# translearn/PaintRL

Measured on NVIDIA B200. Metric: batched env steps/sec, higher is better.
Workload: dtype f64

## Files before the change

### paintrl_b200/csrc/paintrl_capi.cu

```cuda
#include <algorithm>
#include <cmath>
#include <cstdio>
#include <cstring>
#include <numeric>
#include <string>
#include <vector>

#include "../../include/paintrl.h"
#include "paintrl_kernels.cuh"
#include "paintrl_raster.cuh"
#include "paintrl_param.cuh"
#include "paintrl_policy.cuh"
#include "paintrl_learn.cuh"

using namespace paintrl;

static const int kFusedBelowEnvs = 16384;

namespace {

thread_local std::string g_error;

int fail(int code, const std::string &msg) {
    g_error = msg;
// ... 47 lines not shown
        if (e == cudaSuccess) ptrs.push_back(*out);
        return e;
    }
    size_t static_bytes() const {
        size_t n = 0;
        for (const Slab &s : slabs) n += s.used;
        return n;
    }
};

}

struct PaintrlEngine {
    int device = 0;
    int num_envs = 0;
    int color = 0;
    DevPack pk{};
    DevConfig cfg{};
    DeviceArena arena;
    EnvState *states = nullptr;
    MoveOut *moves = nullptr;
    EnvStat *env_stats = nullptr;
    unsigned *bits = nullptr;
    int16_t *thick = nullptr;
    unsigned *grid_cnt = nullptr;
    unsigned long long *stats = nullptr;
    ShotPoses *shots = nullptr;
    unsigned *last_mask = nullptr;
    bool paint_normal = false;
    unsigned *ready = nullptr;
    int carveout_percent = -1;
    bool carveout_set = false;
    bool carveout_set_subset = false;
    void *stage_actions = nullptr;
    unsigned char *stage_out = nullptr;
    void *slot_actions[2] = {nullptr, nullptr};
    unsigned char *slot_out[2] = {nullptr, nullptr};
    cudaStream_t copy_in = nullptr, copy_out = nullptr;
    cudaEvent_t ev_in[2] = {nullptr, nullptr}, ev_step[2] = {nullptr, nullptr}, ev_done[2] = {nullptr, nullptr};
    bool slot_pending[2] = {false, false};
    unsigned long long launches = 0;
    double move_cell_planes_mean = 0.0, move_cell_verts_mean = 0.0;
    int move_lanes = 32;
    int move_warps = 4, paint_warps = 1;
    int move_minb = 4;
    void *cold_args = nullptr;
    int fused = -1;
    bool move_fast = true;
    bool force_unstaged = false;
};

namespace {

bool host_ray(const PaintrlPartPack *pack, const double *frm, const double *d, double *t_hit, int *arg_in = nullptr,
              int *arg_out = nullptr) {
    double t_in = -INFINITY, t_out = INFINITY;
    int ai = -1, ao = -1;
    bool outside = false;
    for (int i = 0; i < pack->n_planes; ++i) {
        const double *n = pack->plane_n + 3 * i;
        double den = n[0] * d[0] + n[1] * d[1] + n[2] * d[2];
        double num = pack->plane_off[i] - (n[0] * frm[0] + n[1] * frm[1] + n[2] * frm[2]);
        if (den == 0.0) {
            if (num < 0.0) { outside = true; if (ai < 0) ai = i; }
            continue;
        }
// ... 629 lines not shown
    }
    return PAINTRL_OK;
}

template <bool SUBSET>
int launch_step(PaintrlHandle h, const EnvSel &sel, const StepIO &io, void *stream) {
    const int n = sel.n;
    const void *actions_dev = io.actions;
    bool &carveout_done = SUBSET ? h->carveout_set_subset : h->carveout_set;
    CUDA_TRY(cudaSetDevice(h->device));
    if (h->paint_normal) {
        cudaStream_t ns = as_stream(stream);
        const int threads = 128;
        move_kernel<32, 4, false, SUBSET><<<(n * 32 + threads - 1) / threads, threads, 0, ns>>>(h->pk, h->cfg, env_arrays(h), h->num_envs, actions_dev, sel);
        int rc = launch_check(h, "move_kernel");
        if (rc != PAINTRL_OK) return rc;
        if (h->color == 0) paint_normal_kernel<0, SUBSET><<<n, 32, 0, ns>>>(h->pk, h->cfg, env_arrays(h), h->num_envs, io, (const ColdArgs *)h->cold_args, sel);
        else paint_normal_kernel<1, SUBSET><<<n, 32, 0, ns>>>(h->pk, h->cfg, env_arrays(h), h->num_envs, io, (const ColdArgs *)h->cold_args, sel);
        cudaError_t nerr = cudaGetLastError();
        if (nerr != cudaSuccess) {
            cudaMemsetAsync(h->ready, 0, sizeof(unsigned) * (size_t)h->num_envs, ns);
            return fail(PAINTRL_E_CUDA, std::string("paint_normal_kernel: ") + cudaGetErrorString(nerr));
        }
        h->launches++;
        return PAINTRL_OK;
    }
    const bool use_fused = h->fused >= 0 ? h->fused == 1 : n < kFusedBelowEnvs;
    if (use_fused) {
        const bool staged_f = h->pk.n_words_pad <= kStageWords && !h->force_unstaged;
        const bool ax12f = h->pk.axis0 == 1 && h->pk.axis1 == 2, disc = h->cfg.action_mode == 0;
        const EnvArrays fea = env_arrays(h);
        const ColdArgs *cold = (const ColdArgs *)h->cold_args;
        cudaStream_t fs = as_stream(stream);
#define PAINTRL_FUSED_K(C, ST, AX, DI) step_fused_kernel<C, ST, AX, DI, SUBSET><<<(n + PAINTRL_FUSED_WPB - 1) / PAINTRL_FUSED_WPB, 32 * PAINTRL_FUSED_WPB, 0, fs>>>(h->pk, h->cfg, fea, h->num_envs, io, cold, sel)
#define PAINTRL_FUSED_AD(C, ST)                                                        \
    do {                                                                               \
        if (ax12f && disc) PAINTRL_FUSED_K(C, ST, true, true);                         \
        else if (ax12f) PAINTRL_FUSED_K(C, ST, true, false);                           \
        else if (disc) PAINTRL_FUSED_K(C, ST, false, true);                            \
        else PAINTRL_FUSED_K(C, ST, false, false);                                     \
    } while (0)
        if (h->color == 0) { if (staged_f) PAINTRL_FUSED_AD(0, true); else PAINTRL_FUSED_AD(0, false); }
        else { if (staged_f) PAINTRL_FUSED_AD(1, true); else PAINTRL_FUSED_AD(1, false); }
#undef PAINTRL_FUSED_AD
#undef PAINTRL_FUSED_K
        return launch_check(h, "step_fused_kernel");
    }
    {
        const int threads = h->move_warps * 32;
        cudaStream_t ms = as_stream(stream);
        const int L = h->move_lanes;
        const int mblocks = (int)(((long long)n * L + threads - 1) / threads);
        const bool ax12m = h->pk.axis0 == 1 && h->pk.axis1 == 2;
#define PAINTRL_MOVE(G, MINB)                                                                                              \
    do {                                                                                                                   \
        if (!carveout_done && h->carveout_percent >= 0) {                                                                \
            cudaFuncSetAttribute(move_kernel<G, MINB, true, SUBSET>, cudaFuncAttributePreferredSharedMemoryCarveout, h->carveout_percent);  \
            cudaFuncSetAttribute(move_kernel<G, MINB, false, SUBSET>, cudaFuncAttributePreferredSharedMemoryCarveout, h->carveout_percent); \
        }                                                                                                                  \
        if (ax12m) move_kernel<G, MINB, true, SUBSET><<<mblocks, threads, 0, ms>>>(h->pk, h->cfg, env_arrays(h), h->num_envs, actions_dev, sel);  \
        else move_kernel<G, MINB, false, SUBSET><<<mblocks, threads, 0, ms>>>(h->pk, h->cfg, env_arrays(h), h->num_envs, actions_dev, sel);       \
    } while (0)
#define PAINTRL_MOVE_FAST(G)                                                                                               \
    do {                                                                                                                   \
        if (ax12m && discrete) move_fast_kernel<G, true, true, SUBSET><<<mblocks, threads, 0, ms>>>(h->pk, h->cfg, env_arrays(h), h->num_envs, actions_dev, sel);   \
        else if (ax12m) move_fast_kernel<G, true, false, SUBSET><<<mblocks, threads, 0, ms>>>(h->pk, h->cfg, env_arrays(h), h->num_envs, actions_dev, sel);         \
        else if (discrete) move_fast_kernel<G, false, true, SUBSET><<<mblocks, threads, 0, ms>>>(h->pk, h->cfg, env_arrays(h), h->num_envs, actions_dev, sel);      \
        else move_fast_kernel<G, false, false, SUBSET><<<mblocks, threads, 0, ms>>>(h->pk, h->cfg, env_arrays(h), h->num_envs, actions_dev, sel);                   \
    } while (0)
        const bool discrete = h->cfg.action_mode == 0;
        if (h->move_fast) {
            if (L == 8) PAINTRL_MOVE_FAST(8); else if (L == 16) PAINTRL_MOVE_FAST(16); else PAINTRL_MOVE_FAST(32);
        } else if (h->move_minb == 7) {
            if (L == 8) PAINTRL_MOVE(8, 7); else if (L == 16) PAINTRL_MOVE(16, 7); else PAINTRL_MOVE(32, 7);
        } else {
            if (L == 8) PAINTRL_MOVE(8, 4); else if (L == 16) PAINTRL_MOVE(16, 4); else PAINTRL_MOVE(32, 4);
        }
#undef PAINTRL_MOVE_FAST
// ... 944 lines not shown
```

### paintrl_b200/csrc/paintrl_kernels.cuh

```cuda
#pragma once
#include "paintrl_device.cuh"

namespace paintrl {

struct StepIO {
    const void *actions;
    double *obs, *reward, *penalty, *actual;
    uint8_t *done;
    int32_t *new_texels;
    double *next_obs;
    const int32_t *reset_start_idx;
};

struct EnvSel {
    const int32_t *ids;
    int lo, n;
};

template <bool SUBSET>
__device__ __forceinline__ bool step_env(const EnvSel &sel, int k, int num_envs, int &env) {
    if (!SUBSET) { env = k; return k < num_envs; }
    if (k >= sel.n) return false;
    env = sel.ids ? __ldg(&sel.ids[k]) : sel.lo + k;
    return (unsigned)env < (unsigned)num_envs;
// ... 382 lines not shown
#pragma unroll
        for (int s = 0; s <= NS; ++s) in |= (ball_exact(ws, x, y, z, s) ? 1u : 0u) << s;
    } else {
#pragma unroll
        for (int s = 0; s <= NS; ++s) in |= (e[s] <= 0.f ? 1u : 0u) << s;
    }
    if (!has_last) in &= (1u << NS) - 1u;
    return in;
}

template <typename WS>
__device__ __forceinline__ void ball_flags_at(const DevPack &pk, const ShotsF &c, const WS &ws, int j, float tx, float ty, float tz,
                                              bool has_last, bool &any_shot, bool &possible) {
    float e[NS + 1];
    bool in[NS + 1];
    if (ball_pretest_at(c, tx, ty, tz, e)) {
        const double x = __ldg(&pk.tx[j]), y = __ldg(&pk.ty[j]), z = __ldg(&pk.tz[j]);
#pragma unroll
        for (int s = 0; s <= NS; ++s) in[s] = ball_exact(ws, x, y, z, s);
    } else {
#pragma unroll
        for (int s = 0; s <= NS; ++s) in[s] = e[s] <= 0.f;
    }
    bool prev = has_last && in[NS];
    any_shot = false;
    possible = false;
#pragma unroll
    for (int s = 0; s < NS; ++s) {
        any_shot = any_shot || in[s];
        possible = possible || (in[s] && !prev);
        prev = in[s];
    }
}
template <typename WS>
__device__ __forceinline__ void ball_flags(const DevPack &pk, const ShotsF &c, const WS &ws, int j, bool has_last, bool &any_shot,
                                           bool &possible) {
    ball_flags_at(pk, c, ws, j, __ldg(&pk.fx[j]), __ldg(&pk.fy[j]), __ldg(&pk.fz[j]), has_last, any_shot, possible);
}

template <bool STAGED, int COLOR, typename WS>
__device__ __forceinline__ int stamp_ranges(const DevPack &pk, float lo0, float hi0, float lo1, float hi1, int lane, WS &ws) {
    const float rr = (float)kPaintRadius + 4e-5f;
    int base = 0;
    for (int r0 = 0; r0 < pk.n_rows; r0 += 32) {
        const int r = r0 + lane;
        int wa = 0, wn = 0;
        if (r < pk.n_rows) {
            const float ylo = fmaf((float)r, pk.rel_row_h, pk.rel_row_o1) - 2e-5f, yhi = ylo + pk.rel_row_h + 4e-5f;
            const float dy = fmaxf(0.f, fmaxf(ylo - hi1, lo1 - yhi));
            if (dy <= rr) {
                const float hw = sqrtf(rr * rr - dy * dy) + 4e-5f;
                const float fa = floorf((lo0 - hw - pk.rel_cx_o0) * pk.rel_cx_inv) - 1.f;
                const float fb = floorf((hi0 + hw - pk.rel_cx_o0) * pk.rel_cx_inv) + 1.f;
                if (fb >= 0.f && fa < (float)pk.ncx) {
                    const int ca = (int)fmaxf(fa, 0.f), cb = (int)fminf(fb, (float)(pk.ncx - 1));
                    const int *cs = pk.cell_start + (size_t)r * (pk.ncx + 1);
                    const int i0 = __ldg(cs + ca), i1 = __ldg(cs + cb + 1);
                    if (i1 > i0) {
                        wa = __ldg(&pk.row_word0[r]) + (i0 >> 5);
                        wn = ((i1 - 1) >> 5) - (i0 >> 5) + 1;
                    }
                }
            }
            ws.rowWa[r] = wa;
            ws.rowWn[r] = wn;
        }
        if (STAGED) {
            int incl = wn;
#pragma unroll
            for (int o = 1; o < 32; o <<= 1) {
                const int u = __shfl_up_sync(kFull, incl, o);
                if (lane >= o) incl += u;
            }
            const int at = base + incl - wn;
            for (int t = 0; t < wn; ++t) ws.cand[at + t] = (uint16_t)(wa + t);
            base += __shfl_sync(kFull, incl, 31);
        }
    }
    __syncwarp();
    return base;
}

template <bool STAGED, typename WS, typename BodyFn>
__device__ __forceinline__ void for_each_stamp_word(const DevPack &pk, int lane, const WS &ws, int n_cand, BodyFn body) {
    if constexpr (STAGED) {
        for (int k = 0; k < n_cand; ++k) body((int)ws.cand[k]);
    } else {
        for (int r0 = 0; r0 < pk.n_rows; r0 += 32) {
            const int r = r0 + lane;
            const int wa = r < pk.n_rows ? ws.rowWa[r] : 0, wn = r < pk.n_rows ? ws.rowWn[r] : 0;
            unsigned m = __ballot_sync(kFull, wn > 0);
            while (m) {
                const int src = __ffs(m) - 1;
                m &= m - 1;
                const int a = __shfl_sync(kFull, wa, src), n = __shfl_sync(kFull, wn, src);
                for (int w = a; w < a + n; ++w) body(w);
            }
        }
    }
}

template <int COLOR, bool STAGED, typename WS, typename BITS>
__device__ __forceinline__ void stamp(const DevPack &pk, const Ax &ax, const BITS &bits, int16_t *thick, unsigned *grid_cnt, bool has_last,
                                      int lane, WS &ws, int &n_new_out, int &n_possible_out, bool &dirty_out PAINTRL_PROF_PARAM) {
    ShotsF c;
#pragma unroll
    for (int s = 0; s <= NS; ++s) {
        c.x[s] = (float)(cen(ws, s, 0) - pk.org0);
        c.y[s] = (float)(cen(ws, s, 1) - pk.org1);
        c.z[s] = (float)(cen(ws, s, 2) - pk.org2);
    }
    float lo0 = INFINITY, hi0 = -INFINITY, lo1 = INFINITY, hi1 = -INFINITY;
#pragma unroll
    for (int s = 0; s < NS; ++s) {
        const float c0 = ax.a0 == 0 ? c.x[s] : (ax.a0 == 1 ? c.y[s] : c.z[s]);
        const float c1 = ax.a1 == 0 ? c.x[s] : (ax.a1 == 1 ? c.y[s] : c.z[s]);
        lo0 = fminf(lo0, c0); hi0 = fmaxf(hi0, c0);
        lo1 = fminf(lo1, c1); hi1 = fmaxf(hi1, c1);
    }
    PAINTRL_PROF(17, lane == 0);
    const int n_cand = stamp_ranges<STAGED, COLOR>(pk, lo0, hi0, lo1, hi1, lane, ws);
    PAINTRL_PROF(18, lane == 0);

    double rmax[NS];
    if (COLOR == 1) {
#pragma unroll
        for (int s = 0; s < NS; ++s) rmax[s] = -1.0;
        for_each_stamp_word<STAGED>(pk, lane, ws, n_cand, [&](int w) {
            const int j = w * 32 + lane;
            const unsigned in = ball_mask(pk, c, ws, j, false);
            if (in) {
                const double x = __ldg(&pk.tx[j]), y = __ldg(&pk.ty[j]), z = __ldg(&pk.tz[j]);
#pragma unroll
                for (int s = 0; s < NS; ++s) {
                    if (in & (1u << s)) {
                        const double dx = x - cen(ws, s, 0), dy = y - cen(ws, s, 1), dz = z - cen(ws, s, 2);
                        rmax[s] = fmax(rmax[s], dx * dx + dy * dy + dz * dz);
                    }
                }
            }
        });
#pragma unroll
        for (int s = 0; s < NS; ++s) rmax[s] = sqrt(warp_max(rmax[s]));
        if (lane < NS) {
// ... 19 lines not shown
                m &= m - 1;
                const int a = __shfl_sync(kFull, wa, src), n = __shfl_sync(kFull, wn, src);
                for (int w0 = a; w0 < a + n; w0 += kBatch) {
                    float tx[kBatch], ty[kBatch], tz[kBatch];
                    unsigned old[kBatch];
#pragma unroll
                    for (int q = 0; q < kBatch; ++q) {
                        const int w = min(w0 + q, a + n - 1);
                        const int j = w * 32 + lane;
                        tx[q] = __ldg(&pk.fx[j]); ty[q] = __ldg(&pk.fy[j]); tz[q] = __ldg(&pk.fz[j]);
                        old[q] = bits.ld(w);
                    }
#pragma unroll
                    for (int q = 0; q < kBatch; ++q) {
                        const int w = w0 + q;
                        if (w >= a + n) break;
                        const int j = w * 32 + lane;
                        bool any_shot, possible;
                        ball_flags_at(pk, c, ws, j, tx[q], ty[q], tz[q], has_last, any_shot, possible);
                        const unsigned uni = __ballot_sync(kFull, any_shot);
                        if (uni == 0u) continue;
                        n_possible += __popc(__ballot_sync(kFull, possible));
                        const unsigned flipped = uni & ~old[q];
                        if (flipped) {
                            n_new += __popc(flipped);
                            if (lane == 0) bits.st(w, old[q] | uni);
                            any |= flipped;
                            if (grid_cnt && ((flipped >> lane) & 1u)) atomicAdd(grid_cnt + __ldg(&pk.gcell[j]), 1u);
                        }
                    }
                }
            }
        }
    } else if (COLOR == 0) {
        for_each_stamp_word<STAGED>(pk, lane, ws, n_cand, [&](int w) {
            const int j = w * 32 + lane;
            bool any_shot, possible;
            ball_flags(pk, c, ws, j, has_last, any_shot, possible);
            const unsigned uni = __ballot_sync(kFull, any_shot);
            if (uni == 0u) return;
            n_possible += __popc(__ballot_sync(kFull, possible));
            const unsigned old = bits.ld(w);
            __syncwarp();
            const unsigned flipped = uni & ~old;
            if (flipped) {
                n_new += __popc(flipped);
                if (lane == 0) bits.st(w, old | uni);
                any |= flipped;
                if (grid_cnt && ((flipped >> lane) & 1u)) atomicAdd(grid_cnt + __ldg(&pk.gcell[j]), 1u);
            }
        });
    } else {
        for_each_stamp_word<STAGED>(pk, lane, ws, n_cand, [&](int w) {
            const int j = w * 32 + lane;
            const unsigned in = ball_mask(pk, c, ws, j, has_last);
            const unsigned shots = in & ((1u << NS) - 1u);
            const unsigned uni = __ballot_sync(kFull, shots != 0u);
            if (uni == 0u) return;
            const unsigned prev = ((shots << 1) | (in >> NS)) & ((1u << NS) - 1u);
            n_possible += __popc(__ballot_sync(kFull, (shots & ~prev) != 0u));
            bool fl = false;
            if (shots) {
                const int sv0 = (int)__ldcg(&thick[j]);
                int sv = sv0;
                const double x = __ldg(&pk.tx[j]), y = __ldg(&pk.ty[j]), z = __ldg(&pk.tz[j]);
#pragma unroll 1
                for (int s = 0; s < NS; ++s) {
                    if ((shots & (1u << s)) && sv > 0) {
                        const double dx = x - cen(ws, s, 0), dy = y - cen(ws, s, 1), dz = z - cen(ws, s, 2);
                        const double d2 = dx * dx + dy * dy + dz * dz;
                        const double qa = kHsiTargetMax * (1.0 - d2 * ws.hsi_r[NS + s]);
                        const double qf = floor(qa);
                        int quantity = (int)qf + 1;
                        if (!(qa > 1e-9 && qa - qf > 1e-9 && (qf + 1.0) - qa > 1e-9)) {
                            const double ratio = sqrt(d2) / ws.hsi_r[s];
                            quantity = (int)(kHsiTargetMax * (1.0 - ratio * ratio)) + 1;
                        }
                        sv -= quantity;
                        n_new += quantity;
                    }
                }
                if (sv != sv0) {
                    __stcg(&thick[j], (int16_t)sv);
// ... 634 lines not shown
        gst->quat[3] = quat[3];
        reinterpret_cast<double2 *>(&gst->last_angle)[0] = make_double2(new_angle, fabs(new_angle - last_angle));
        gst->term_counter = term_counter;
        gst->flags = flags;
        mv->counts = term_counter - counter_before;
        if (!FUSED) asm volatile("st.release.gpu.global.u32 [%0], %1;" ::"l"(ea.ready + env), "r"(kReadyMoved) : "memory");
    }
    PAINTRL_TRACE_MARK(env, 1, grp.gl == 0);
    return false;
}

#ifndef PAINTRL_MOVE_FAST_MINB
#define PAINTRL_MOVE_FAST_MINB 7
#endif
template <int G, bool AX12, bool DISCRETE, bool SUBSET = false>
__global__ void __launch_bounds__(kWarpsPerBlock * 32, PAINTRL_MOVE_FAST_MINB)
move_fast_kernel(DevPack pk, DevConfig cfg, EnvArrays ea, int num_envs, const void *actions, EnvSel sel) {
    asm volatile("griddepcontrol.launch_dependents;");
    const int k = (blockIdx.x * blockDim.x + threadIdx.x) / G;
    int env;
    if (!step_env<SUBSET>(sel, k, num_envs, env)) return;
    if (cfg.debug_bail_mod > 0 && env % cfg.debug_bail_mod == 0) {
        if ((threadIdx.x & (G - 1)) == 0) asm volatile("st.release.gpu.global.u32 [%0], %1;" ::"l"(ea.ready + env), "r"(kReadyBailed) : "memory");
        return;
    }
    move_fast_body<G, AX12, DISCRETE, false>(pk, cfg, ea, env, k, actions, nullptr, nullptr);
}

struct ColdArgs { DevPack pk; DevConfig cfg; EnvArrays ea; };
__device__ __noinline__ void move_generic_cold(const ColdArgs *ca, int env, int row, const void *actions) {
    move_body<32, false>(ca->pk, ca->cfg, ca->ea, env, row, actions);
}

template <int COLOR, bool STAGED, bool AX12, bool FUSED = false, bool DISCRETE = false, bool NORMAL = false>
__device__ __forceinline__ void paint_body(const DevPack &pk, const DevConfig &cfg, const EnvArrays &ea, int env, int row, const StepIO &io,
                                           WarpScratch<STAGED> &ws, const ColdArgs *cold, NormalScratch *ns = nullptr) {
    const Ax ax = make_ax<AX12>(pk.axis0, pk.axis1);
    typedef WarpScratch<STAGED> WS;
    const int lane = threadIdx.x & 31;
    PAINTRL_PROF_BEGIN(env, 15, 32)
    PAINTRL_TRACE_MARK(env, 2, lane == 0);
    PAINTRL_TRACE_SM(env, 7, lane == 0);
    unsigned *gbits = bits_of(pk, ea, env), *grid_cnt = grid_cnt_of(pk, ea, env);
    int16_t *thick = thick_of(pk, ea, env);
    const unsigned plane_bytes = (unsigned)pk.n_words_pad * 4u;
    const bool late_copy = FUSED && STAGED && !NORMAL && cfg.start_order;
    auto issue_copy = [&]() {
        if (STAGED && lane == 0) {
            mbar_init(&ws.bar, 1);
            mbar_expect_tx(&ws.bar, plane_bytes);
            bulk_g2s(ws.sbits, gbits, plane_bytes, &ws.bar);
        }
    };
    const unsigned tid = blockIdx.x * blockDim.x + threadIdx.x, nthreads = gridDim.x * blockDim.x;
    if (FUSED && !cfg.start_order) l2_prefetch_tables(pk, tid, nthreads);
    if (!late_copy) issue_copy();
    int bailed = 0;
    if (FUSED) {
        if (lane < 8) reinterpret_cast<double2 *>(&ws.st)[lane] = __ldcg(reinterpret_cast<const double2 *>(&ea.states[env]) + lane);
        if (cfg.start_order) l2_prefetch_tables(pk, tid, nthreads);
        __syncwarp();
        if (cfg.debug_bail_mod > 0 && env % cfg.debug_bail_mod == 0) bailed = 1;
        else bailed = move_fast_body<32, AX12, DISCRETE, true>(pk, cfg, ea, env, row, io.actions, &ws.st, &ws.mv) ? 1 : 0;
        __syncwarp();
        if (late_copy) issue_copy();
    } else {
        if (lane == 0) {
            const unsigned *flag = ea.ready + env;
            unsigned v;
// ... 21 lines not shown
            double2 *dst = lane < 8 ? reinterpret_cast<double2 *>(&ws.st) + lane : reinterpret_cast<double2 *>(&ws.mv) + (lane - 8);
            *dst = __ldcg(src);
        }
        __syncwarp();
    }
    if (STAGED && !late_copy) mbar_wait(&ws.bar, 0);
    PAINTRL_TRACE_MARK(env, 4, lane == 0);
    PAINTRL_PROF(16, lane == 0);
    const Bits<STAGED> bits = {gbits, ws.sbits};
    EnvState &st = ws.st;
    const Vec3 cur_p = {st.pose[0], st.pose[1], st.pose[2]};
    const bool fast4 = (cfg.obs_mode == 0 || cfg.obs_mode == 3) && cfg.obs_grad == 4;
    if (fast4) {
        row_ranks(pk, ax, comp(cur_p, ax.a0), lane, ws);
        const int prow = pose_row(pk, comp(cur_p, ax.a1));
        if (prow >= 0 && prow < pk.n_rows) {
            const int w0 = __ldg(&pk.row_word0[prow]), w1 = __ldg(&pk.row_word0[prow + 1]);
            const char *ky = reinterpret_cast<const char *>(axis_table(pk, ax.a1) + (size_t)w0 * 32);
            for (int k = lane; k < 2 * (w1 - w0); k += 32) prefetch_l1(ky + (size_t)k * 128);
        }
    }
    if (STAGED && late_copy) mbar_wait(&ws.bar, 0);
    PAINTRL_PROF(15, lane == 0);

    const bool has_last = (st.flags & kFlagHasLast) != 0;
    int n_new, n_possible;
    bool dirty;
    if (NORMAL) {
        const double *src = reinterpret_cast<const double *>(&ea.shots[env]);
        for (int i = lane; i < kPaintPerAction * 7; i += 32) (&ns->pos[0][0])[i] = __ldcg(src + i);
        __syncwarp();
        stamp_normal<COLOR>(pk, cfg, ax, bits, thick, grid_cnt, ea.last_mask + (size_t)env * pk.n_words_pad, lane, ws, *ns, n_new, n_possible, dirty);
    } else {
        stamp<COLOR, STAGED>(pk, ax, bits, thick, grid_cnt, has_last, lane, ws, n_new, n_possible, dirty PAINTRL_PROF_PASS);
    }
    PAINTRL_PROF(19, lane == 0);

    int flags = st.flags | kFlagHasLast;
    const double succeeded = (COLOR == 0) ? (double)n_new : (double)n_new / 255.0;
    if ((ws.mv.counts & 0xf) >= kPaintPerAction && n_possible == 0) flags |= kFlagTerminate;
    const double radius = kPaintRadius;
    const double axis1_real = comp(cur_p, ax.a0), axis2_real = comp(cur_p, ax.a1);
    double rate, reward, turn, axis2_in, rel;
    {
        double num = succeeded, den = n_possible ? (double)n_possible : 1.0;
        if (lane == 1) den = 100.0;
        if (lane == 2) { num = st.angle_diff; den = kPi; }
        if (lane == 3) { num = axis2_real - pk.range1_min + radius; den = pk.range1_max - pk.range1_min + 2 * radius; }
        if (lane == 4) { num = axis2_real - pk.range1_min; den = pk.range1_max - pk.range1_min; }
        double q = 0.0;
        if (num != 0.0) q = num / den;
        rate = n_possible ? __shfl_sync(kFull, q, 0) : 0.0;
        reward = __shfl_sync(kFull, q, 1);
        turn = __shfl_sync(kFull, q, 2);
        axis2_in = __shfl_sync(kFull, q, 3);
        rel = __shfl_sync(kFull, q, 4);
    }
    const double total_reward = st.total_reward + reward;
    double penalty = 0.2;
    if (cfg.overlap_penalty) penalty += 0.1 * (1 - rate);
    if (cfg.turning_penalty) penalty += 0.1 * turn;
    const double actual = reward - penalty;
    const int step_counter = st.step_counter + 1;
    int gi;
    {
        const double scaled = rel * pk.grid_granularity;
        gi = !(scaled > -1.0) ? 0 : (scaled >= (double)pk.grid_granularity ? pk.grid_granularity - 1 : (int)scaled);
// ... 99 lines not shown
    __syncwarp();
    if (lane < 8) reinterpret_cast<double2 *>(&ea.states[env])[lane] = reinterpret_cast<const double2 *>(&st)[lane];
    if (STAGED && lane == 0) bulk_wait_read();
    PAINTRL_PROF(26, lane == 0);
    PAINTRL_TRACE_MARK(env, 5, lane == 0);
}

#ifndef PAINTRL_PAINT_OCC
#define PAINTRL_PAINT_OCC 28
#endif
template <int COLOR, bool STAGED, bool AX12, int WPB, bool SUBSET = false>
__global__ void __launch_bounds__(WPB * 32, (STAGED ? PAINTRL_PAINT_OCC : 16) / WPB)
paint_kernel(DevPack pk, DevConfig cfg, EnvArrays ea, int num_envs, StepIO io, const ColdArgs *cold, EnvSel sel) {
    __shared__ WarpScratch<STAGED> scratch[WPB];
    const int warp = threadIdx.x >> 5;
    const int k = blockIdx.x * WPB + warp;
    int env;
    if (!step_env<SUBSET>(sel, k, num_envs, env)) return;
    paint_body<COLOR, STAGED, AX12>(pk, cfg, ea, env, k, io, scratch[warp], cold);
}

template <int COLOR, bool SUBSET = false>
__global__ void __launch_bounds__(32, 14)
paint_normal_kernel(DevPack pk, DevConfig cfg, EnvArrays ea, int num_envs, StepIO io, const ColdArgs *cold, EnvSel sel) {
    __shared__ WarpScratch<true> scratch[1];
    __shared__ NormalScratch nscratch[1];
    const int k = blockIdx.x;
    int env;
    if (!step_env<SUBSET>(sel, k, num_envs, env)) return;
    paint_body<COLOR, true, false, false, false, true>(pk, cfg, ea, env, k, io, scratch[0], cold, &nscratch[0]);
}

#ifndef PAINTRL_FUSED_WPB
#define PAINTRL_FUSED_WPB 1
#endif
template <int COLOR, bool STAGED, bool AX12, bool DISCRETE, bool SUBSET = false>
__global__ void __launch_bounds__(32 * PAINTRL_FUSED_WPB, (STAGED ? PAINTRL_PAINT_OCC : 16) / PAINTRL_FUSED_WPB)
step_fused_kernel(DevPack pk, DevConfig cfg, EnvArrays ea, int num_envs, StepIO io, const ColdArgs *cold, EnvSel sel) {
    __shared__ WarpScratch<STAGED> scratch[PAINTRL_FUSED_WPB];
    const int warp = threadIdx.x >> 5;
    const int k = blockIdx.x * PAINTRL_FUSED_WPB + warp;
    int env;
    if (!step_env<SUBSET>(sel, k, num_envs, env)) return;
    paint_body<COLOR, STAGED, AX12, true, DISCRETE>(pk, cfg, ea, env, k, io, scratch[warp], cold);
}

__global__ void __launch_bounds__(kWarpsPerBlock * 32)
reset_kernel(DevPack pk, DevConfig cfg, EnvArrays ea, int num_envs, const int32_t *env_ids, int n, const int32_t *start_idx,
             const double *set_pos, const double *set_normal, double *obs_out, int mode ) {
    const Ax ax = make_ax<false>(pk.axis0, pk.axis1);
    __shared__ WarpScratch<false> scratch[kWarpsPerBlock];
    const int lane = threadIdx.x & 31, warp = threadIdx.x >> 5;
    const int k = blockIdx.x * kWarpsPerBlock + warp;
    if (k >= n) return;
    const int env = env_ids ? env_ids[k] : k;
    if ((unsigned)env >= (unsigned)num_envs) return;
    unsigned *gbits = bits_of(pk, ea, env), *grid_cnt = grid_cnt_of(pk, ea, env);
    int16_t *thick = thick_of(pk, ea, env);
    if (lane == 0) ea.ready[env] = 0u;
    EnvState st;
    load_state(&ea.states[env], st);
    if (mode == 0) {
        int idx = start_idx ? start_idx[k] : auto_start_index(pk, cfg, env, st.episode);
        idx = min(max(idx, 0), pk.n_starts - 1);
        clear_planes(pk, Bits<false>{gbits, nullptr}, gbits, thick, grid_cnt, lane);
        if (ea.last_mask)
            for (int w = lane; w < pk.n_words_pad; w += 32) ea.last_mask[(size_t)env * pk.n_words_pad + w] = 0u;
        state_reset(pk, st, idx);
    } else {
        robot_reset(st, set_pos + 3 * k, set_normal + 3 * k);
    }
    __syncwarp();
    const Bits<false> bits = {gbits, nullptr};
    Vec3 pose = {st.pose[0], st.pose[1], st.pose[2]};
    PAINTRL_PROF_BEGIN(65535, 0, 0)
    write_observation(pk, ax, cfg, bits, grid_cnt, pose, lane, scratch[warp], obs_out ? obs_out + (size_t)k * cfg.obs_dim : nullptr,
                      nullptr PAINTRL_PROF_PASS);
// ... 126 lines not shown
```

### profiles/timeline.py

```python
#!/usr/bin/env python
import argparse, ctypes, os, sys
sys.path.insert(0, os.path.dirname(os.path.dirname(os.path.abspath(__file__))))
import numpy as np
import torch
import bench
from paintrl_b200 import _capi
from paintrl_b200.batched_env import BatchedPaintEnv
from paintrl_b200.config import EnvConfig

ap = argparse.ArgumentParser()
ap.add_argument('--envs', type=int, default=4096)
ap.add_argument('--workload', default='c2')
ap.add_argument('--steps', type=int, default=40)
ap.add_argument('--out', default=None)
ap.add_argument('--uniform', action='store_true', help='every environment at start point 0 with action 0: identical work per warp, what is left is scheduling')
ap.add_argument('--no-flush', action='store_true')
args = ap.parse_args()
w = bench.WORKLOADS[args.workload]
cfg = EnvConfig(w['extra'], auto_reset=True, seed=1234, **w['kw'])
dev = torch.device('cuda:0')
env = BatchedPaintEnv(args.envs, cfg, device=dev, texture_size=w.get('texture', (240, 240)))
lib = _capi.lib()
lib.paintrl_debug_trace.restype = ctypes.c_int
lib.paintrl_debug_trace.argtypes = [ctypes.c_void_p, ctypes.c_int]
gen = torch.Generator(device=dev); gen.manual_seed(1234)
acts = torch.randint(0, cfg.discrete_granularity, (args.steps, args.envs), generator=gen, device=dev, dtype=torch.int64)
env.reset(torch.randint(0, env.n_starts, (args.envs,), generator=gen, device=dev, dtype=torch.int32))
if args.uniform:
    acts.zero_()
    env.reset(torch.zeros(args.envs, dtype=torch.int32, device=dev))
    args.steps = min(args.steps, 6)
flush = torch.empty(512 << 20, dtype=torch.uint8, device=dev)
for i in range(args.steps):
    if not args.no_flush:
        flush.fill_(i & 255)
    env.step(acts[i])
torch.cuda.synchronize()
n = min(args.envs, 65536)
tr = np.zeros((n, 8), dtype=np.uint64)
if lib.paintrl_debug_trace(tr.ctypes.data, n) == 0:
    raise SystemExit('not a trace build: PAINTRL_TRACE=1 python -m paintrl_b200.build --force')
t = tr[:, :6].astype(np.int64)
t0 = t[:, 0].min()
t = (t - t0) / 1e3
names = ['move start', 'move end', 'paint start', 'paint dependency resolved', 'paint inputs loaded', 'paint end']
print('%s, %d envs: last step, microseconds since the first move warp started' % (args.workload, n))
for k, nm in enumerate(names):
    c = t[:, k]
    print('  %-28s min %7.2f  p10 %7.2f  median %7.2f  p90 %7.2f  max %7.2f' % (nm, c.min(), np.percentile(c, 10), np.median(c), np.percentile(c, 90), c.max()))
dm, dp = t[:, 1] - t[:, 0], t[:, 5] - t[:, 4]
for nm, d in (('move duration per warp', dm), ('paint duration per warp (after inputs)', dp)):
    print('  %-40s min %6.2f  p10 %6.2f  median %6.2f  p90 %6.2f  p99 %6.2f  max %6.2f' % (nm, d.min(), np.percentile(d, 10), np.median(d), np.percentile(d, 90), np.percentile(d, 99), d.max()))
sm_m, sm_p = (tr[:, 6] & 0xffff).astype(int), tr[:, 7].astype(int)
cnt = ((tr[:, 6] >> 16) & 0xffffffff).astype(np.int64)
max_planes, max_verts = ((tr[:, 6] >> 48) & 0xff).astype(int), ((tr[:, 6] >> 56) & 0xff).astype(int)
off, full, verify, attempts = cnt & 0xf, (cnt >> 8) & 0xff, (cnt >> 16) & 0xff, (cnt >> 24) & 0x7f
slow = np.argsort(-dm)[:24]
print('  slowest move warps: duration us / off-part sub-steps / full plane scans (two-kernel step) or cached-pair tests (one-kernel step) / verify passes / cell attempts')
print('   ' + '  '.join('%.1f/%d/%d/%d/%d' % (dm[i], off[i], full[i], verify[i], attempts[i]) for i in slow))
print('  their SMs: ' + ' '.join(str(sm_m[i]) for i in slow) + '   start us: ' + ' '.join('%.1f' % t[i, 0] for i in slow))
print('  their largest plane list / vertex list: ' + ' '.join('%d/%d' % (max_planes[i], max_verts[i]) for i in slow))
for lo_, hi_ in ((0, 17), (17, 33), (33, 65), (65, 129), (129, 256)):
    sel = (max_planes >= lo_) & (max_planes < hi_)
    if sel.any():
        print('  move duration, largest plane list in [%d, %d): n %5d  median %6.2f  p90 %6.2f  max %6.2f' % (lo_, hi_, sel.sum(), np.median(dm[sel]), np.percentile(dm[sel], 90), dm[sel].max()))
for lo_, hi_ in ((0, 17), (17, 33), (33, 65), (65, 256)):
    sel = (max_verts >= lo_) & (max_verts < hi_)
    if sel.any():
        print('  move duration, largest vertex list in [%d, %d): n %5d  median %6.2f  p90 %6.2f  max %6.2f' % (lo_, hi_, sel.sum(), np.median(dm[sel]), np.percentile(dm[sel], 90), dm[sel].max()))
pose = env.get_state()['pose'].cpu().numpy()[:n]
pk = env.pack
a0, a1 = pk.axes
r = pk.ranges
n0 = (pose[:, a0] - r[0, 0]) / (r[0, 1] - r[0, 0]); n1 = (pose[:, a1] - r[1, 0]) / (r[1, 1] - r[1, 0])
print('  their poses after the step (fraction of the part extent along axis 0 / axis 1): ' + ' '.join('%.2f/%.2f' % (n0[i], n1[i]) for i in slow))
edge = np.minimum(np.minimum(n0, 1 - n0), np.minimum(n1, 1 - n1))
for lo_, hi_ in ((-9, 0.02), (0.02, 0.05), (0.05, 0.1), (0.1, 0.2), (0.2, 0.6)):
    sel = (edge >= lo_) & (edge < hi_)
    if sel.any():
        print('  move duration, distance to the bounding box edge in [%.2f, %.2f): n %5d  median %6.2f  p90 %6.2f  max %6.2f   paint median %6.2f' % (lo_, hi_, sel.sum(), np.median(dm[sel]), np.percentile(dm[sel], 90), dm[sel].max(), np.median(dp[sel])))
for k in range(5, 16):
    sel = attempts == k
    if sel.any():
        print('  move duration, %2d cell attempts: n %5d  median %6.2f  p90 %6.2f  max %6.2f' % (k, sel.sum(), np.median(dm[sel]), np.percentile(dm[sel], 90), dm[sel].max()))
for k in range(0, 6):
    sel = verify == k
    if sel.any():
        print('  move duration, %d verify passes: n %5d  median %6.2f  p90 %6.2f  max %6.2f' % (k, sel.sum(), np.median(dm[sel]), np.percentile(dm[sel], 90), dm[sel].max()))
for nm, sel in (('no slow path', (full == 0) & (verify == 0)), ('verify only', (full == 0) & (verify > 0)), ('full scans', full > 0)):
    if sel.any():
        print('  move duration, %-12s: n %5d  median %6.2f  p90 %6.2f  max %6.2f' % (nm, sel.sum(), np.median(dm[sel]), np.percentile(dm[sel], 90), dm[sel].max()))
for k in range(6):
    sel = off == k
    if sel.any():
        print('  move duration, %d off-part sub-steps: n %5d  median %6.2f  p90 %6.2f  max %6.2f' % (k, sel.sum(), np.median(dm[sel]), np.percentile(dm[sel], 90), dm[sel].max()))
print('  move: warps per SM min %d max %d; last move end per SM: min %.2f median %.2f max %.2f' % (
    np.bincount(sm_m).min(), np.bincount(sm_m).max(), *np.percentile([t[sm_m == s, 1].max() for s in np.unique(sm_m)], [0, 50, 100])))
print('  paint: warps per SM min %d max %d; last paint end per SM: min %.2f median %.2f max %.2f' % (
    np.bincount(sm_p).min(), np.bincount(sm_p).max(), *np.percentile([t[sm_p == s, 5].max() for s in np.unique(sm_p)], [0, 50, 100])))
for nm, a, b in (('move', t[:, 0], t[:, 1]), ('paint', t[:, 4], t[:, 5])):
    grid = np.linspace(0, t[:, 5].max(), 41)
    inflight = [(int(((a <= g) & (b > g)).sum())) for g in grid]
    print('  %s warps in flight every %.1f us: %s' % (nm, grid[1], ' '.join(str(v) for v in inflight)))
if args.out:
    np.save(args.out, tr)
```

Before: 80.31 million.

## Share stamp work across warps in fused kernel via shared-memory work slots

Raises the fused kernel from one warp per block to many warps per block (staged path) with dynamic shared memory. Each owner warp publishes its stamp candidate list in a shared slot. Idle or finished warps claim chunks of words atomically, so one env's heavy stamping no longer becomes the tail. Warps without an env prefetch tables into L2. The cost is atomics, nanosleep polling and coarser block scheduling, and a whole block stays resident until every warp finishes.

```diff
diff --git a/paintrl_b200/csrc/paintrl_capi.cu b/paintrl_b200/csrc/paintrl_capi.cu
--- a/paintrl_b200/csrc/paintrl_capi.cu
+++ b/paintrl_b200/csrc/paintrl_capi.cu
@@ -103,6 +103,8 @@
     int carveout_percent = -1;
     bool carveout_set = false;
     bool carveout_set_subset = false;
+    bool fused_smem_set = false;
+    bool fused_smem_set_subset = false;
     void *stage_actions = nullptr;
     unsigned char *stage_out = nullptr;
     void *slot_actions[2] = {nullptr, nullptr};
@@ -798,7 +800,13 @@
         const EnvArrays fea = env_arrays(h);
         const ColdArgs *cold = (const ColdArgs *)h->cold_args;
         cudaStream_t fs = as_stream(stream);
-#define PAINTRL_FUSED_K(C, ST, AX, DI) step_fused_kernel<C, ST, AX, DI, SUBSET><<<(n + PAINTRL_FUSED_WPB - 1) / PAINTRL_FUSED_WPB, 32 * PAINTRL_FUSED_WPB, 0, fs>>>(h->pk, h->cfg, fea, h->num_envs, io, cold, sel)
+        bool &smem_done = SUBSET ? h->fused_smem_set_subset : h->fused_smem_set;
+#define PAINTRL_FUSED_K(C, ST, AX, DI)                                                                                     \
+    do {                                                                                                               \
+        constexpr int smem = (int)sizeof(FusedSmem<ST>);                                                               \
+        if (!smem_done) cudaFuncSetAttribute(step_fused_kernel<C, ST, AX, DI, SUBSET>, cudaFuncAttributeMaxDynamicSharedMemorySize, smem); \
+        step_fused_kernel<C, ST, AX, DI, SUBSET><<<(n + fused_wpb(ST) - 1) / fused_wpb(ST), 32 * fused_wpb(ST), smem, fs>>>(h->pk, h->cfg, fea, h->num_envs, io, cold, sel); \
+    } while (0)
 #define PAINTRL_FUSED_AD(C, ST)                                                        \
     do {                                                                               \
         if (ax12f && disc) PAINTRL_FUSED_K(C, ST, true, true);                         \
@@ -810,6 +818,7 @@
         else { if (staged_f) PAINTRL_FUSED_AD(1, true); else PAINTRL_FUSED_AD(1, false); }
 #undef PAINTRL_FUSED_AD
 #undef PAINTRL_FUSED_K
+        smem_done = true;
         return launch_check(h, "step_fused_kernel");
     }
     {
diff --git a/paintrl_b200/csrc/paintrl_kernels.cuh b/paintrl_b200/csrc/paintrl_kernels.cuh
--- a/paintrl_b200/csrc/paintrl_kernels.cuh
+++ b/paintrl_b200/csrc/paintrl_kernels.cuh
@@ -438,11 +438,6 @@
         prev = in[s];
     }
 }
-template <typename WS>
-__device__ __forceinline__ void ball_flags(const DevPack &pk, const ShotsF &c, const WS &ws, int j, bool has_last, bool &any_shot,
-                                           bool &possible) {
-    ball_flags_at(pk, c, ws, j, __ldg(&pk.fx[j]), __ldg(&pk.fy[j]), __ldg(&pk.fz[j]), has_last, any_shot, possible);
-}
 
 template <bool STAGED, int COLOR, typename WS>
 __device__ __forceinline__ int stamp_ranges(const DevPack &pk, float lo0, float hi0, float lo1, float hi1, int lane, WS &ws) {
@@ -487,6 +482,135 @@
     return base;
 }
 
+template <typename WS>
+__device__ __forceinline__ ShotsF shots_f(const DevPack &pk, const WS &ws) {
+    ShotsF c;
+#pragma unroll
+    for (int s = 0; s <= NS; ++s) {
+        c.x[s] = (float)(cen(ws, s, 0) - pk.org0);
+        c.y[s] = (float)(cen(ws, s, 1) - pk.org1);
+        c.z[s] = (float)(cen(ws, s, 2) - pk.org2);
+    }
+    return c;
+}
+
+template <typename WS, typename BITS>
+__device__ __forceinline__ void stamp_word_rgb(const DevPack &pk, const ShotsF &c, const WS &ws, const BITS &bits, unsigned *grid_cnt,
+                                               bool has_last, int lane, int w, int &n_new, int &n_possible, unsigned &any) {
+    const int j = w * 32 + lane;
+    bool any_shot, possible;
+    ball_flags_at(pk, c, ws, j, __ldg(&pk.fx[j]), __ldg(&pk.fy[j]), __ldg(&pk.fz[j]), has_last, any_shot, possible);
+    const unsigned uni = __ballot_sync(kFull, any_shot);
+    if (uni == 0u) return;
+    n_possible += __popc(__ballot_sync(kFull, possible));
+    const unsigned old = bits.ld(w);
+    __syncwarp();
+    const unsigned flipped = uni & ~old;
+    if (flipped) {
+        n_new += __popc(flipped);
+        if (lane == 0) bits.st(w, old | uni);
+        any |= flipped;
+        if (grid_cnt && ((flipped >> lane) & 1u)) atomicAdd(grid_cnt + __ldg(&pk.gcell[j]), 1u);
+    }
+}
+
+struct StampSlot {
+    unsigned *grid_cnt;
+    int state;
+    int n_cand;
+    int next;
+    int done;
+    int n_new, n_possible;
+    unsigned any;
+};
+constexpr int kSlotIdle = 0, kSlotOpen = 1, kSlotClosed = 2;
+#ifndef PAINTRL_STAMP_CHUNK
+#define PAINTRL_STAMP_CHUNK 2
+#endif
+struct StampShare {
+    StampSlot *slot;
+    int *closed;
+};
+
+__device__ __forceinline__ int ld_volatile(const int *p) { return *reinterpret_cast<const volatile int *>(p); }
+
+__device__ __forceinline__ int2 claim_words(StampSlot &slot, int n_cand, int lane) {
+    int k0 = 0;
+    if (lane == 0) k0 = atomicAdd(&slot.next, PAINTRL_STAMP_CHUNK);
+    k0 = __shfl_sync(kFull, k0, 0);
+    return make_int2(k0, min(k0 + PAINTRL_STAMP_CHUNK, n_cand));
+}
+
+template <typename WS, typename BITS>
+__device__ __forceinline__ int stamp_claimed(const DevPack &pk, const ShotsF &c, const WS &ws, const BITS &bits, unsigned *grid_cnt,
+                                             bool has_last, int lane, StampSlot &slot, int n_cand, int2 r, int &n_new,
+                                             int &n_possible, unsigned &any) {
+    int cnt = 0;
+    while (r.x < r.y) {
+        int nk = 0;
+        if (lane == 0) nk = atomicAdd(&slot.next, PAINTRL_STAMP_CHUNK);
+        for (int k = r.x; k < r.y; ++k) stamp_word_rgb(pk, c, ws, bits, grid_cnt, has_last, lane, (int)ws.cand[k], n_new, n_possible, any);
+        cnt += r.y - r.x;
+        nk = __shfl_sync(kFull, nk, 0);
+        r = make_int2(nk, min(nk + PAINTRL_STAMP_CHUNK, n_cand));
+    }
+    return cnt;
+}
+
+template <typename WS>
+__device__ __forceinline__ bool help_stamp(const DevPack &pk, WS &ws, StampSlot &slot, int lane) {
+    const int n_cand = slot.n_cand;
+    if (__shfl_sync(kFull, ld_volatile(&slot.next), 0) >= n_cand) return false;
+    int2 r = claim_words(slot, n_cand, lane);
+    if (r.x >= r.y) return false;
+    const ShotsF c = shots_f(pk, ws);
+    const bool has_last = (ws.st.flags & kFlagHasLast) != 0;
+    const Bits<true> bits = {nullptr, ws.sbits};
+    unsigned *grid_cnt = slot.grid_cnt;
+    int n_new = 0, n_possible = 0;
+    unsigned any = 0;
+    const int cnt = stamp_claimed(pk, c, ws, bits, grid_cnt, has_last, lane, slot, n_cand, r, n_new, n_possible, any);
+    if (lane == 0) fence_async_smem();
+    __syncwarp();
+    if (lane == 0) {
+        if (n_new) atomicAdd(&slot.n_new, n_new);
+        if (n_possible) atomicAdd(&slot.n_possible, n_possible);
+        if (any) atomicOr(&slot.any, any);
+        __threadfence_block();
+        atomicAdd(&slot.done, cnt);
+    }
+    return true;
+}
+
+template <int WPB, typename WS>
+__device__ __forceinline__ void stamp_helper_loop(const DevPack &pk, WS *scratch, StampSlot *slots, const int *closed, int n_owners,
+                                                  int lane) {
+    static_assert(WPB <= 32, "one lane per slot");
+    unsigned ns = 64;
+    for (;;) {
+        const int state = lane < WPB ? ld_volatile(&slots[lane].state) : kSlotIdle;
+        unsigned open = __ballot_sync(kFull, state == kSlotOpen);
+        bool worked = false;
+        if (open) {
+            __threadfence_block();
+            __syncwarp();
+            while (open) {
+                const int o = __ffs(open) - 1;
+                open &= open - 1;
+                worked |= help_stamp(pk, scratch[o], slots[o], lane);
+            }
+        } else if (__shfl_sync(kFull, ld_volatile(closed), 0) >= n_owners) {
+            return;
+        }
+        if (worked) {
+            ns = 64;
+        } else {
+            __nanosleep(ns);
+            ns = min(2u * ns, 512u);
+        }
+    }
+}
+
 template <bool STAGED, typename WS, typename BodyFn>
 __device__ __forceinline__ void for_each_stamp_word(const DevPack &pk, int lane, const WS &ws, int n_cand, BodyFn body) {
     if constexpr (STAGED) {
@@ -506,16 +630,11 @@
     }
 }
 
-template <int COLOR, bool STAGED, typename WS, typename BITS>
+template <int COLOR, bool STAGED, bool SHARE = false, typename WS, typename BITS>
 __device__ __forceinline__ void stamp(const DevPack &pk, const Ax &ax, const BITS &bits, int16_t *thick, unsigned *grid_cnt, bool has_last,
-                                      int lane, WS &ws, int &n_new_out, int &n_possible_out, bool &dirty_out PAINTRL_PROF_PARAM) {
-    ShotsF c;
-#pragma unroll
-    for (int s = 0; s <= NS; ++s) {
-        c.x[s] = (float)(cen(ws, s, 0) - pk.org0);
-        c.y[s] = (float)(cen(ws, s, 1) - pk.org1);
-        c.z[s] = (float)(cen(ws, s, 2) - pk.org2);
-    }
+                                      int lane, WS &ws, int &n_new_out, int &n_possible_out, bool &dirty_out, StampShare sh PAINTRL_PROF_PARAM) {
+    static_assert(!SHARE || (COLOR == 0 && STAGED), "stamp sharing: staged RGB only");
+    const ShotsF c = shots_f(pk, ws);
     float lo0 = INFINITY, hi0 = -INFINITY, lo1 = INFINITY, hi1 = -INFINITY;
 #pragma unroll
     for (int s = 0; s < NS; ++s) {
@@ -601,23 +720,38 @@
                 }
             }
         }
+    } else if (SHARE) {
+        StampSlot &slot = *sh.slot;
+        if (lane == 0) {
+            slot.grid_cnt = grid_cnt;
+            slot.n_cand = n_cand;
+            __threadfence_block();
+            *reinterpret_cast<volatile int *>(&slot.state) = kSlotOpen;
+        }
+        const int own = stamp_claimed(pk, c, ws, bits, grid_cnt, has_last, lane, slot, n_cand, claim_words(slot, n_cand, lane), n_new,
+                                      n_possible, any);
+        if (lane == 0) {
+            *reinterpret_cast<volatile int *>(&slot.state) = kSlotClosed;
+            atomicAdd(sh.closed, 1);
+        }
+        if (own < n_cand) {
+            unsigned ns = 32;
+            for (;;) {
+                int d = 0;
+                if (lane == 0) d = ld_volatile(&slot.done);
+                if (__shfl_sync(kFull, d, 0) >= n_cand - own) break;
+                __nanosleep(ns);
+                ns = min(2u * ns, 256u);
+            }
+            __threadfence_block();
+            __syncwarp();
+            n_new += ld_volatile(&slot.n_new);
+            n_possible += ld_volatile(&slot.n_possible);
+            any |= (unsigned)ld_volatile(reinterpret_cast<const int *>(&slot.any));
+        }
     } else if (COLOR == 0) {
         for_each_stamp_word<STAGED>(pk, lane, ws, n_cand, [&](int w) {
-            const int j = w * 32 + lane;
-            bool any_shot, possible;
-            ball_flags(pk, c, ws, j, has_last, any_shot, possible);
-            const unsigned uni = __ballot_sync(kFull, any_shot);
-            if (uni == 0u) return;
-            n_possible += __popc(__ballot_sync(kFull, possible));
-            const unsigned old = bits.ld(w);
-            __syncwarp();
-            const unsigned flipped = uni & ~old;
-            if (flipped) {
-                n_new += __popc(flipped);
-                if (lane == 0) bits.st(w, old | uni);
-                any |= flipped;
-                if (grid_cnt && ((flipped >> lane) & 1u)) atomicAdd(grid_cnt + __ldg(&pk.gcell[j]), 1u);
-            }
+            stamp_word_rgb(pk, c, ws, bits, grid_cnt, has_last, lane, w, n_new, n_possible, any);
         });
     } else {
         for_each_stamp_word<STAGED>(pk, lane, ws, n_cand, [&](int w) {
@@ -1318,9 +1452,9 @@
     move_body<32, false>(ca->pk, ca->cfg, ca->ea, env, row, actions);
 }
 
-template <int COLOR, bool STAGED, bool AX12, bool FUSED = false, bool DISCRETE = false, bool NORMAL = false>
+template <int COLOR, bool STAGED, bool AX12, bool FUSED = false, bool DISCRETE = false, bool NORMAL = false, bool SHARE = false>
 __device__ __forceinline__ void paint_body(const DevPack &pk, const DevConfig &cfg, const EnvArrays &ea, int env, int row, const StepIO &io,
-                                           WarpScratch<STAGED> &ws, const ColdArgs *cold, NormalScratch *ns = nullptr) {
+                                           WarpScratch<STAGED> &ws, const ColdArgs *cold, NormalScratch *ns = nullptr, StampShare sh = {}) {
     const Ax ax = make_ax<AX12>(pk.axis0, pk.axis1);
     typedef WarpScratch<STAGED> WS;
     const int lane = threadIdx.x & 31;
@@ -1408,7 +1542,11 @@
         __syncwarp();
         stamp_normal<COLOR>(pk, cfg, ax, bits, thick, grid_cnt, ea.last_mask + (size_t)env * pk.n_words_pad, lane, ws, *ns, n_new, n_possible, dirty);
     } else {
-        stamp<COLOR, STAGED>(pk, ax, bits, thick, grid_cnt, has_last, lane, ws, n_new, n_possible, dirty PAINTRL_PROF_PASS);
+        stamp<COLOR, STAGED, SHARE>(pk, ax, bits, thick, grid_cnt, has_last, lane, ws, n_new, n_possible, dirty, sh PAINTRL_PROF_PASS);
+#ifdef PAINTRL_TRACE
+        if (SHARE && lane == 0 && env < 65536)
+            g_trace[env][7] |= ((unsigned long long)(unsigned)sh.slot->done << 32) | ((unsigned long long)(unsigned)sh.slot->n_cand << 48);
+#endif
     }
     PAINTRL_PROF(19, lane == 0);
 
@@ -1574,17 +1712,41 @@
 }
 
 #ifndef PAINTRL_FUSED_WPB
-#define PAINTRL_FUSED_WPB 1
+#define PAINTRL_FUSED_WPB 28
 #endif
+__host__ __device__ constexpr int fused_wpb(bool staged) { return staged ? PAINTRL_FUSED_WPB : 1; }
+
+template <bool STAGED>
+struct FusedSmem {
+    WarpScratch<STAGED> scratch[fused_wpb(STAGED)];
+    StampSlot slot[fused_wpb(STAGED)];
+    int closed;
+};
+
 template <int COLOR, bool STAGED, bool AX12, bool DISCRETE, bool SUBSET = false>
-__global__ void __launch_bounds__(32 * PAINTRL_FUSED_WPB, (STAGED ? PAINTRL_PAINT_OCC : 16) / PAINTRL_FUSED_WPB)
+__global__ void __launch_bounds__(32 * fused_wpb(STAGED), (STAGED ? PAINTRL_PAINT_OCC : 16) / fused_wpb(STAGED))
 step_fused_kernel(DevPack pk, DevConfig cfg, EnvArrays ea, int num_envs, StepIO io, const ColdArgs *cold, EnvSel sel) {
-    __shared__ WarpScratch<STAGED> scratch[PAINTRL_FUSED_WPB];
-    const int warp = threadIdx.x >> 5;
-    const int k = blockIdx.x * PAINTRL_FUSED_WPB + warp;
+    constexpr int WPB = fused_wpb(STAGED);
+    constexpr bool SHARE = STAGED && COLOR == 0 && WPB > 1;
+    extern __shared__ __align__(128) unsigned char fused_smem[];
+    FusedSmem<STAGED> &sm = *reinterpret_cast<FusedSmem<STAGED> *>(fused_smem);
+    const int warp = threadIdx.x >> 5, lane = threadIdx.x & 31;
+    const int k = blockIdx.x * WPB + warp;
     int env;
-    if (!step_env<SUBSET>(sel, k, num_envs, env)) return;
-    paint_body<COLOR, STAGED, AX12, true, DISCRETE>(pk, cfg, ea, env, k, io, scratch[warp], cold);
+    const bool has_env = step_env<SUBSET>(sel, k, num_envs, env);
+    int n_owners = 0;
+    if constexpr (SHARE) {
+        if (lane == 0) sm.slot[warp] = StampSlot{nullptr, kSlotIdle, 0, 0, 0, 0, 0, 0u};
+        if (threadIdx.x == 0) sm.closed = 0;
+        n_owners = __syncthreads_count(has_env && lane == 0);
+    }
+    if (has_env) {
+        paint_body<COLOR, STAGED, AX12, true, DISCRETE, false, SHARE>(pk, cfg, ea, env, k, io, sm.scratch[warp], cold, nullptr,
+                                                                     StampShare{&sm.slot[warp], &sm.closed});
+    } else {
+        l2_prefetch_tables(pk, blockIdx.x * blockDim.x + threadIdx.x, gridDim.x * blockDim.x);
+    }
+    if constexpr (SHARE) stamp_helper_loop<WPB>(pk, sm.scratch, sm.slot, &sm.closed, n_owners, lane);
 }
 
 __global__ void __launch_bounds__(kWarpsPerBlock * 32)
diff --git a/profiles/timeline.py b/profiles/timeline.py
--- a/profiles/timeline.py
+++ b/profiles/timeline.py
@@ -51,7 +51,8 @@
 dm, dp = t[:, 1] - t[:, 0], t[:, 5] - t[:, 4]
 for nm, d in (('move duration per warp', dm), ('paint duration per warp (after inputs)', dp)):
     print('  %-40s min %6.2f  p10 %6.2f  median %6.2f  p90 %6.2f  p99 %6.2f  max %6.2f' % (nm, d.min(), np.percentile(d, 10), np.median(d), np.percentile(d, 90), np.percentile(d, 99), d.max()))
-sm_m, sm_p = (tr[:, 6] & 0xffff).astype(int), tr[:, 7].astype(int)
+sm_m, sm_p = (tr[:, 6] & 0xffff).astype(int), (tr[:, 7] & 0xffff).astype(int)
+helped, cand = ((tr[:, 7] >> 32) & 0xffff).astype(np.int64), ((tr[:, 7] >> 48) & 0xffff).astype(np.int64)
 cnt = ((tr[:, 6] >> 16) & 0xffffffff).astype(np.int64)
 max_planes, max_verts = ((tr[:, 6] >> 48) & 0xff).astype(int), ((tr[:, 6] >> 56) & 0xff).astype(int)
 off, full, verify, attempts = cnt & 0xf, (cnt >> 8) & 0xff, (cnt >> 16) & 0xff, (cnt >> 24) & 0x7f
@@ -98,6 +99,10 @@
     np.bincount(sm_m).min(), np.bincount(sm_m).max(), *np.percentile([t[sm_m == s, 1].max() for s in np.unique(sm_m)], [0, 50, 100])))
 print('  paint: warps per SM min %d max %d; last paint end per SM: min %.2f median %.2f max %.2f' % (
     np.bincount(sm_p).min(), np.bincount(sm_p).max(), *np.percentile([t[sm_p == s, 5].max() for s in np.unique(sm_p)], [0, 50, 100])))
+if cand.sum():
+    last = np.argsort(-t[:, 5])[:24]
+    print('  stamp words: %d candidate, %d (%.1f %%) stamped by helpers; environments helped %d of %d; last 24 paint ends: helped / candidate words %s' % (
+        cand.sum(), helped.sum(), 100.0 * helped.sum() / cand.sum(), (helped > 0).sum(), n, ' '.join('%d/%d' % (helped[i], cand[i]) for i in last)))
 for nm, a, b in (('move', t[:, 0], t[:, 1]), ('paint', t[:, 4], t[:, 5])):
     grid = np.linspace(0, t[:, 5].max(), 41)
     inflight = [(int(((a <= g) & (b > g)).sum())) for g in grid]
```

After: 81.72 million (median of 6 runs). 1.02x the previous value.
